# NethermindEth/starkpack-winterfell

Hardware: AMD Instinct MI355X
Metric: trace-LDE + Merkle-commit field-ops/s (wall-clock ms in ms_per_step), 2^20x8 f64 trace blowup=8 (higher is better)
Workload: dtype u64 (Goldilocks, Montgomery form) + u32 (BLAKE3)

## Files before the change

### starkpack-winterfell_amd/csrc/context.hip

```cpp
#include "wf_internal.hpp"

#include <atomic>

#include "field.hpp"

using namespace wf;

static thread_local char g_err[512] = "";

std::atomic<uint64_t> g_fail_epoch{0};
uint64_t fail_epoch() { return g_fail_epoch.load(std::memory_order_relaxed); }

int fail(int code, const char *fmt, ...) {
    g_fail_epoch.fetch_add(1, std::memory_order_relaxed);
    va_list ap;
    va_start(ap, fmt);
    vsnprintf(g_err, sizeof(g_err), fmt, ap);
    va_end(ap);
    return code;
}

const char *last_error_text() { return g_err; }

wf_tuning tuning_from_env() {
// ... 2 lines not shown
    if (!on || strcmp(on, "1") != 0) return t;
    if (const char *e = getenv("WF_EXP_MAX_DIGIT")) {
        const int v = atoi(e);
        if (v >= 4 && v <= 11) t.max_digit = (uint32_t)v;
    }
    t.no_specialized = getenv("WF_EXP_NO_SPECIALIZED") != nullptr;
    t.full_tiles = getenv("WF_EXP_FULL_TILES") != nullptr;
    t.no_fused_hash = getenv("WF_EXP_NO_FUSED_HASH") != nullptr;
    t.no_chunked = getenv("WF_EXP_NO_CHUNKED") != nullptr;
    t.persistent_always = getenv("WF_EXP_PERSISTENT_ALWAYS") != nullptr;
    t.no_persistent = getenv("WF_EXP_NO_PERSISTENT") != nullptr;
    if (const char *e = getenv("WF_EXP_MERKLE_L2_MIN")) {
        const int v = atoi(e);
        if (v >= 10 && v <= 30) t.merkle_l2_min = (uint32_t)v;
    }
    t.no_pipeline = getenv("WF_EXP_NO_PIPELINE") != nullptr;
    t.no_tail_pack = getenv("WF_EXP_NO_TAIL_PACK") != nullptr;
    t.no_coset_inner = getenv("WF_EXP_NO_COSET_INNER") != nullptr;
    t.no_gtab = getenv("WF_EXP_NO_GTAB") != nullptr;
    t.no_staged_chunks = getenv("WF_EXP_NO_STAGED_CHUNKS") != nullptr;
    t.no_gtab1 = getenv("WF_EXP_NO_GTAB1") != nullptr;
    t.no_ftab = getenv("WF_EXP_NO_FTAB") != nullptr;
    t.no_gtab1_wide = getenv("WF_EXP_NO_GTAB1_WIDE") != nullptr;
    t.gtab1_f64 = getenv("WF_EXP_GTAB1_F64") != nullptr;
    if (const char *e = getenv("WF_EXP_WIDE_TI")) {
        const int v = atoi(e);
        if (v == 1 || v == 2 || v == 4 || v == 8) t.wide_ti = (uint32_t)v;
    }
    if (const char *e = getenv("WF_EXP_PIPELINE_MIN_BYTES")) {
        const long long v = atoll(e);
        if (v >= 0 && v <= (1ll << 40)) t.pipeline_min_bytes = (size_t)v;
    }
    if (const char *e = getenv("WF_EXP_FAIL_AFTER_SEGMENT")) {
        const int v = atoi(e);
        if (v >= 0 && v < 4096) t.fail_after_segment = v;
    }
    if (const char *e = getenv("WF_EXP_GRIND_WINDOW_LOG2")) {
        const int v = atoi(e);
        if (v >= 2 && v <= 30) t.grind_window_log2 = (uint32_t)v;
    }
    if (const char *e = getenv("WF_EXP_GRIND_WINDOW_CAP_LOG2")) {
        const int v = atoi(e);
        if (v >= 2 && v <= 30) t.grind_window_cap_log2 = (uint32_t)v;
    }
    return t;
}
// ... 395 lines not shown
```

### starkpack-winterfell_amd/csrc/path.hip

```cpp
#include "wf_internal.hpp"

#include "kernels.hpp"
#include "keccak_dev.hpp"
#include "keccak_kernels.hpp"
#include "merkle_plan.hpp"
#include "rescue_kernels.hpp"
#include "rescue_jive_kernels.hpp"
#include "griffin_dev.hpp"
#include "seg_kernels.hpp"
#include "col_kernels.hpp"
#include "fri_kernels.hpp"
#include "tables.hpp"

using namespace wf;

#if defined(WF_EXPERIMENTS) && defined(WF_EXP_STAMPS)
static unsigned long long *g_exp_stamps = nullptr;
static unsigned long long *exp_stamps_buffer() {
    if (!g_exp_stamps && hipMalloc(&g_exp_stamps, 4096 * 8 * 8) == hipSuccess) (void)hipMemset(g_exp_stamps, 0, 4096 * 8 * 8);
    return g_exp_stamps;
}
extern "C" int wf_exp_stamps_read(unsigned long long *out, int clear) {
    if (!g_exp_stamps) return -1;
    if (hipMemcpy(out, g_exp_stamps, 4096 * 8 * 8, hipMemcpyDeviceToHost) != hipSuccess) return -2;
// ... 181 lines not shown
    return true;
}

template <class F>
struct SegDesc {
    typedef typename F::T T;
    const T *in;
    T *work;
    T *out;
    uint32_t logN, n_seg, n_cosets;
    bool rows_out;
    void *leaves = nullptr;
    uint32_t hash_epr = 0;
    uint32_t digest_words = 8;
    bool *fused = nullptr;
    const TableSet *pre;
    const T *fin_tab = nullptr;
    bool pad_traces = false;
    bool pad_in_kernel = false;
    uint32_t base_cols, total_base_cols, coset0;
    uint64_t row_width, trace_lde_elems;
    uint32_t seg0 = 0, seg_cnt = 0;
    int phase = 0;
};

template <class F>
static int run_seg_transform(wf_ctx *ctx, hipStream_t st, const SegDesc<F> &d) {
    typedef typename F::T T;
    const bool inverse = !d.rows_out;
    TableSet *tw;
    int rc = root_tables<F>(ctx, d.logN, inverse, &tw);
    if (rc) return rc;
    const Plan plan = seg_plan<F>(d.logN, d.n_seg, ctx->tune.max_digit, ctx->tune.full_tiles);
    const uint64_t N = (uint64_t)1 << d.logN;

    SegArgs<F> a;
    memset(&a, 0, sizeof(a));
    a.logN = d.logN;
    a.n_seg = d.n_seg;
    a.n_cosets = d.n_cosets;
    a.tw = as_pow2l<F>(*tw);
    if (d.pre) {
        a.pre = as_pow2l<F>(*d.pre);
        a.pre_lo_stride = d.pre->lo_stride;
        a.pre_hi_stride = d.pre->hi_stride;
    }
    a.base_cols = d.base_cols;
// ... 59 lines not shown
            a.dst = d.work;
            a.src_shared = 0;
            a.pre_on = 0;
            a.scale_on = first ? 1 : 0;
            a.scale = inv_n;
        }
        a.src += run_off;
        a.dst += run_off;
        a.n_seg = run_cnt;
        uint32_t threads;
        size_t lds;
        rc = seg_launch_dims<F>(a.logD, threads, lds, false);
        if (rc) return rc;
        const uint64_t grid = (uint64_t)n_groups * run_cnt * a.O * a.I;
        if (grid > 0x7FFFFFFFull) return fail(WF_ERR_ARG, "problem too large for one launch (%llu groups)", (unsigned long long)grid);
        auto coset_inner = [&](uint32_t cosets, uint64_t tiles_per_coset) -> uint32_t {
            if (!(d.rows_out && first) || ctx->tune.no_coset_inner || cosets < 2 || (cosets & (cosets - 1)) || (tiles_per_coset & 63)) return 0u;
            uint32_t lc = 0;
            while ((1u << lc) < cosets) lc++;
            return lc + 1;
        };
        prof_mark(ctx, st, tag_s);
        const bool spec_ok = F::BYTES == 8 && !packed && threads * 2 == (1u << a.logD) && !ctx->tune.no_specialized;
        const void *kern = nullptr;
        if (spec_ok) {
            constexpr bool F8 = F::BYTES == 8;
            switch (a.logD) {
                case 10: kern = d.rows_out ? (const void *)k_seg_strided<F, 1, false, F8 ? 10 : 0> : (const void *)k_seg_strided<F, 0, false, F8 ? 10 : 0>; break;
                case 9: kern = d.rows_out ? (const void *)k_seg_strided<F, 1, false, F8 ? 9 : 0> : (const void *)k_seg_strided<F, 0, false, F8 ? 9 : 0>; break;
                default: break;
            }
        }
        uint32_t ti = 0;
        if (F::BYTES == 8 && !packed && plan.n_pass >= 3 && a.logD >= 4 && a.logD <= 8 && ctx->tune.wide_ti != 1) {
            ti = ctx->tune.wide_ti ? ctx->tune.wide_ti : 2u;
            while (ti > 1 && (ti > a.I || ((size_t)(ti * SegCfg<F>::S + 2 + ti) << a.logD) * sizeof(T) > 80 * 1024)) ti >>= 1;
            if (ti < 2 || ((1u << a.logD) * ti * SegCfg<F>::S) / 16 < 64) ti = 0;
        }
        a.coset_inner = coset_inner(n_groups, ((uint64_t)run_cnt * a.O * a.I) / (ti ? ti : 1u));
        a.fout_tab = nullptr;
        if (!ti && d.rows_out && first && !packed && a.pre_on && !a.scale_on && d.logN <= 20 && !ctx->tune.no_gtab1 &&
            (F::BYTES == 16 || ctx->tune.gtab1_f64)) {
            rc = pass_factor_table<F>(ctx, d.logN, a.logD, (uint32_t)(d.logN - a.logD), inverse, &a.fout_tab);
            if (rc) return rc;
        }
        if (ti) {
// ... 166 lines not shown
            int rcq = ensure_tickets(ctx, st);
            if (rcq) return rcq;
            a.tile_counters = (uint32_t *)ctx->tickets.p;
#if defined(WF_EXPERIMENTS) && defined(WF_EXP_STAMPS)
            a.stamps = exp_stamps_buffer();
#endif
            void *kargs[] = {&a};
            HIP_TRY(hipLaunchKernel(kern, dim3((uint32_t)std::min<uint64_t>(tickets, resident)), dim3(threads), kargs, lds_p, st));
            if (chunked) {
                HIP_TRY(hipGetLastError());
                launch_merge_chunks(st, ctx->hash_tmp.p, n_chunks, launch_rows, d.leaves, a.digest_words);
            }
        } else if (d.rows_out && packed)
            hipLaunchKernelGGL((k_seg_last<F, SEG_OUT_ROWS, true>), dim3((uint32_t)grid), dim3(threads), lds, st, a);
        else {
            const void *kern = d.rows_out ? (const void *)k_seg_last<F, SEG_OUT_ROWS> : (const void *)k_seg_last<F, SEG_OUT_SEG>;
            constexpr bool F8 = F::BYTES == 8;
            if (F8 && threads * 2 == (1u << a.logD) && !ctx->tune.no_specialized) {
                if (a.logD == 10)
                    kern = d.rows_out ? (const void *)k_seg_last<F, SEG_OUT_ROWS, false, F8 ? 10 : 0> : (const void *)k_seg_last<F, SEG_OUT_SEG, false, F8 ? 10 : 0>;
                else if (a.logD == 9)
                    kern = d.rows_out ? (const void *)k_seg_last<F, SEG_OUT_ROWS, false, F8 ? 9 : 0> : (const void *)k_seg_last<F, SEG_OUT_SEG, false, F8 ? 9 : 0>;
            }
            if (lds > 64 * 1024) HIP_TRY(hipFuncSetAttribute(kern, hipFuncAttributeMaxDynamicSharedMemorySize, 160 * 1024));
            void *kargs[] = {&a};
            HIP_TRY(hipLaunchKernel(kern, dim3((uint32_t)grid), dim3(threads), kargs, lds, st));
        }
        HIP_TRY(hipGetLastError());
    }
    return 0;
}

template <class F>
static int run_xpose(wf_ctx *ctx, hipStream_t st, bool to_seg, const void *src, void *dst, uint64_t R, uint32_t W,
                     uint32_t total_base_cols, uint32_t n_seg, uint32_t seg0 = 0, uint32_t seg_cnt = 0) {
    if (seg_cnt == 0) seg_cnt = n_seg - seg0;
    XposeArgs<F> x;
    x.seg0 = seg0;
    x.src = (const typename F::T *)src;
    x.dst = (typename F::T *)dst;
    x.R = R;
    x.W = W;
    x.total_base_cols = total_base_cols;
    constexpr uint32_t RPB = XPOSE_TILES * 256 / SegCfg<F>::S;
    const uint64_t grid = (uint64_t)seg_cnt * ((R + RPB - 1) / RPB);
    if (grid > 0x7FFFFFFFull) return fail(WF_ERR_ARG, "problem too large for one launch");
// ... 205 lines not shown
    if (d_leaves) {
        if (!hashed) {
            prof_mark(ctx, st, "hash_rows");
            rc = run_hash_rows<F>(ctx, st, d_lde, Nrows * row_width, Nrows, (uint32_t)row_width, base_cols, p->n_traces, d_leaves, p->hasher, p->digest_bytes);
            if (rc) return rc;
        }
        if (d_nodes) {
            prof_mark(ctx, st, "merkle");
            rc = run_merkle(ctx, st, d_leaves, Nrows, d_nodes, p->hasher, p->digest_bytes);
            if (rc) return rc;
        }
    }
    prof_mark(ctx, st, "between_calls");
    return 0;
}

template <class F>
static int trace_commit_dev(wf_ctx *ctx, const wf_params *p, const void *d_trace, void *d_polys, void *d_lde,
                            void *d_leaves, void *d_nodes, hipStream_t st, hipEvent_t input_read = nullptr) {
    PathBufs<F> b;
    int rc = path_buffers<F>(ctx, p, b);
    if (rc) return rc;
    const uint64_t R = (uint64_t)1 << p->log2_trace_len;
    rc = run_xpose<F>(ctx, st, true, d_trace, b.segA, R, p->ext_degree, b.total_base_cols, b.n_seg);
    if (rc) return rc;
    if (input_read) HIP_TRY(hipEventRecord(input_read, st));
    SegDesc<F> d;
    memset(&d, 0, sizeof(d));
    d.in = b.segA;
    d.work = b.segA;
    d.out = b.segB;
    d.logN = p->log2_trace_len;
    d.n_seg = b.n_seg;
    d.n_cosets = 1;
    d.rows_out = false;
    rc = run_seg_transform<F>(ctx, st, d);
    if (rc) return rc;
    rc = run_xpose<F>(ctx, st, false, b.segB, d_polys, R, p->ext_degree, b.total_base_cols, b.n_seg);
    if (rc) return rc;
    return evaluate_and_commit<F>(ctx, st, p, b, d_lde, d_leaves, d_nodes);
}

template <class F>
static int trace_commit_pipelined_impl(wf_ctx *ctx, const wf_params *p, const void *const *cols_in, void *d_stage, void *d_polys,
                                       void *d_lde, void *d_leaves, void *d_nodes, hipStream_t st, void *const *polys_out) {
    typedef typename F::T T;
    constexpr uint32_t S = SegCfg<F>::S;
    PathBufs<F> b;
    int rc = path_buffers<F>(ctx, p, b);
    if (rc) return rc;
    const uint64_t R = (uint64_t)1 << p->log2_trace_len;
    const size_t colb = R * sizeof(T), TC = b.total_base_cols;
    if (!ctx->copy_stream) HIP_TRY(hipStreamCreateWithFlags(&ctx->copy_stream, hipStreamNonBlocking));
    while (ctx->seg_events.size() < (size_t)b.n_seg + 1) {
        hipEvent_t e;
        HIP_TRY(hipEventCreateWithFlags(&e, hipEventDisableTiming));
        ctx->seg_events.push_back(e);
    }
// ... 591 lines not shown
```

### starkpack-winterfell_amd/csrc/seg_kernels.hpp

```cpp
#pragma once

#include <hip/hip_runtime.h>
#include <stdint.h>

#include "field.hpp"
#include "kernels.hpp"

#ifndef WF_EXPERIMENTS
#undef WF_EXP_SKIP_LOAD
#undef WF_EXP_SKIP_NTT
#undef WF_EXP_SKIP_STORE
#undef WF_EXP_LOCAL_STORE
#undef WF_EXP_STAMPS
#endif

namespace wf {

template <class F>
struct SegCfg {
    static constexpr uint32_t S = 64 / F::BYTES;
    static constexpr uint32_t HP = S / 2;
    static constexpr bool RADIX16 = F::BYTES == 8;
    static constexpr bool RADIX8 = F::BYTES == 16;
    static constexpr uint32_t LOAD_BATCH = F::BYTES == 8 ? 8 : 4;
// ... 540 lines not shown
        T w8[4];
#pragma unroll
        for (int j = 0; j < 4; j++) w8[j] = twd[j * (D >> 3)];
        for (uint32_t r = radix8_rounds(logD); r > 0; r--) {
            seg_round8<F, LANES>(x, twd, w8, logD, cur, nthr, threadIdx.x);
            cur -= 3;
            __syncthreads();
        }
    }
    T w4 = F::one();
    if (logD >= 2) w4 = twd[D >> 2];
    while (cur > 0) {
        if (cur >= 2) {
            seg_round4<F, DIR, false, LANES>(x, twd, w4, logD, cur, nthr, threadIdx.x);
            cur -= 2;
        } else {
            seg_round2<F, LANES>(x, logD, nthr, threadIdx.x);
            cur = 0;
        }
        __syncthreads();
    }
}

template <class F, int EVAL, bool PACKED = false, int LOGD = 0>
__global__ void WF_TILE_BOUNDS(LOGD, 1024) k_seg_strided(SegArgs<F> a) {
    typedef typename F::T T;
    if (LOGD) a.logD = LOGD;
    const uint32_t NT = tile_threads<LOGD>();
    typedef Pair<T> P2;
    constexpr uint32_t S = SegCfg<F>::S, HP = SegCfg<F>::HP;
    constexpr uint32_t hp_shift = HP == 4 ? 2 : 1;
    extern __shared__ __attribute__((aligned(16))) unsigned char smem_raw[];
    const uint32_t D = 1u << a.logD;
    T *x = reinterpret_cast<T *>(smem_raw);
    T *twd = x + (size_t)D * S;
    constexpr bool ONE_TABLE = F::BYTES == 16;
    T *aux = ONE_TABLE ? twd : twd + D;

    uint64_t bid = xcd_group_index(blockIdx.x, gridDim.x);
    const uint32_t logI = ilog2_pow2(a.I), logO = ilog2_pow2(a.O);
    uint32_t c_in = 0;
    if (a.coset_inner) bid = coset_inner_split(bid, a.coset_inner - 1, c_in);
    const uint64_t i = bid & (a.I - 1);
    const uint64_t o = (bid >> logI) & (a.O - 1);
    const uint32_t rest = (uint32_t)(bid >> (logI + logO));
    const uint32_t c = a.coset_inner ? c_in : rest / a.n_seg, g = a.coset_inner ? rest : rest - c * a.n_seg;
    const uint64_t seg_elems = ((uint64_t)1 << a.logN) * S;
    const T *src = a.src + (a.src_shared ? (uint64_t)g : (uint64_t)c * a.seg_stride + g) * seg_elems;
    T *dst = a.dst + ((uint64_t)c * a.seg_stride + g) * seg_elems;

    Pow2L<F> pre = a.pre;
    Pow2L<F> pre_a = a.pre, pre_b = a.pre;
    const uint32_t lane_a = 2 * (threadIdx.x & (HP - 1)), lane_b = lane_a + 1;
    const bool act_a = PACKED && (lane_a & ((1u << a.lg_log) - 1)) < a.total_base_cols && (lane_a >> a.lg_log) < (1u << a.cpr_log);
    const bool act_b = PACKED && (lane_b & ((1u << a.lg_log) - 1)) < a.total_base_cols && (lane_b >> a.lg_log) < (1u << a.cpr_log);
    if (PACKED && a.pre_on) {
        const uint32_t ca = a.coset0 + (c << a.cpr_log) + (act_a ? (lane_a >> a.lg_log) : 0);
        const uint32_t cb = a.coset0 + (c << a.cpr_log) + (act_b ? (lane_b >> a.lg_log) : 0);
        pre_a.lo += (uint64_t)ca * a.pre_lo_stride;
        pre_a.hi += (uint64_t)ca * a.pre_hi_stride;
        pre_b.lo += (uint64_t)cb * a.pre_lo_stride;
        pre_b.hi += (uint64_t)cb * a.pre_hi_stride;
    } else if (a.pre_on) {
        pre.lo += (uint64_t)(a.coset0 + c) * a.pre_lo_stride;
        pre.hi += (uint64_t)(a.coset0 + c) * a.pre_hi_stride;
    }
    const uint32_t nitems = D * HP;
    const uint64_t row0 = ((o << a.logD) << logI) + i;
    const uint32_t step = NT;
    const bool from_regs = !(PACKED && a.pre_on);
    const uint32_t tw_shift = a.logN - a.logD - logI;
    const bool scale_in = !PACKED && a.pre_on;
    const Pow2L<F> pin = scale_in ? pre : a.tw;
    const bool gtab = !PACKED && a.fout_tab != nullptr;
    uint32_t kq[2];
    T fo_a[2], fo_b[2], tw_q[2], fi_a[2], fi_b[2];
#pragma unroll
    for (uint32_t q = 0; q < 2; q++) {
        const uint32_t k = threadIdx.x + q * NT;
        kq[q] = k < D ? k : D - 1;
        if (gtab)
            fo_a[q] = fo_b[q] = a.fout_tab[(i << a.logD) + kq[q]];
        else
            a.tw.fetch(((uint64_t)kq[q] * i) << tw_shift, fo_a[q], fo_b[q]);
        tw_q[q] = a.digit_tw[kq[q]];
        pin.fetch(((uint64_t)kq[q] << logI) + (gtab ? i : 0), fi_a[q], fi_b[q]);
    }
    const bool direct = !PACKED && SegCfg<F>::RADIX16 && a.logD >= 4 && from_regs;
    const uint32_t m16 = D >> 4, l16 = threadIdx.x & (S - 1), j16 = threadIdx.x / S;
    const bool has16 = threadIdx.x < m16 * S;
    T vr[16];
    uint4 r0, r1, r2, r3, r4, r5, r6, r7;
    r0 = r1 = r2 = r3 = r4 = r5 = r6 = r7 = make_uint4(0, 0, 0, 0);
    if (direct) {
        if (has16) {
            const T *pr = src + (row0 + ((uint64_t)j16 << logI)) * S + l16;
            const uint64_t rstep = ((uint64_t)m16 << logI) * S;
#pragma unroll
            for (uint32_t q = 0; q < 16; q++) {
#ifdef WF_EXP_SKIP_LOAD
                vr[q] = src[l16];
#else
                vr[q] = *pr;
#endif
                pr += rstep;
            }
        }
    } else if (from_regs) {
#ifdef WF_EXP_SKIP_LOAD
#define WF_ITEM_PTR(WK) reinterpret_cast<const uint4 *>(src + 2 * ((WK) & (HP - 1)))
#else
#define WF_ITEM_PTR(WK) \
    reinterpret_cast<const uint4 *>(src + (row0 + ((uint64_t)((WK) >> hp_shift) << logI)) * S + 2 * ((WK) & (HP - 1)))
#endif
#define WF_LOAD_ITEM(U, RA, RB)                            \
    do {                                                   \
        const uint32_t wk_ = threadIdx.x + (U) * step;     \
        if (wk_ < nitems) {                                \
            const uint4 *p_ = WF_ITEM_PTR(wk_);            \
            RA = p_[0];                                    \
// ... 104 lines not shown
#ifndef WF_EXP_SKIP_NTT
    seg_lds_ntt<F, EVAL ? 1 : -1, (LOGD ? (1u << LOGD) : 0u)>(x, twd, a.logD, NT, direct ? vr : nullptr, direct);
#else
    if (direct && has16) {
#pragma unroll
        for (uint32_t q = 0; q < 16; q++) x[(q * m16 + j16) * S + l16] = vr[q];
    }
    __syncthreads();
#endif
    if (ONE_TABLE) {
        if (threadIdx.x < D) aux[threadIdx.x] = unpark<F>(fok0);
        if (threadIdx.x + NT < D) aux[threadIdx.x + NT] = unpark<F>(fok1);
        __syncthreads();
    }

    T start_a = F::one(), start_b = F::one();
    if (PACKED && a.pre_on) {
        start_a = pre_a.get(i);
        start_b = pre_b.get(i);
    }
    const uint32_t pstride = NT >> hp_shift, pos0 = threadIdx.x >> hp_shift;
    if (pos0 >= D) return;
    const uint32_t k0 = seg_digit_reverse<F>(pos0, a.logD);
    T *dst_lane = dst + row0 * S + lane_a;
    const uint32_t k_shift = logI + (S == 8 ? 3 : 2);
    for (uint32_t pj = 0; pj < D; pj += pstride) {
        const uint32_t k = k0 | seg_digit_reverse<F>(pj, a.logD);
        P2 v = *reinterpret_cast<P2 *>(x + (pos0 + pj) * S + lane_a);
        const T f = aux[k];
        v.a = F::mul(v.a, f);
        v.b = F::mul(v.b, f);
        if (PACKED && a.pre_on) {
            v.a = F::mul(v.a, start_a);
            v.b = F::mul(v.b, start_b);
        }
#ifdef WF_EXP_SKIP_STORE
        if (*reinterpret_cast<const uint32_t *>(&v.a) == a.logN + 77777u)
#endif
        store_pair(dst_lane + ((uint64_t)k << k_shift), v);
    }
}

template <class F, int EVAL, int TI, int GTAB = 0, int LOGD = 0>
__global__ void __launch_bounds__(1024) k_seg_strided_wide(SegArgs<F> a) {
    if (LOGD) a.logD = LOGD;
    static_assert(SegCfg<F>::RADIX16 && TI >= 2 && (TI & (TI - 1)) == 0, "f64 tiles of 2, 4 or 8 inner positions");
    typedef typename F::T T;
    typedef Pair<T> P2;
    constexpr uint32_t S = SegCfg<F>::S, LANES = TI * S, HPW = LANES / 2;
    constexpr uint32_t LOGS = ilog2_const(S), LOGL = ilog2_const(LANES), LOGTI = ilog2_const(TI), LOGHPW = ilog2_const(HPW);
    extern __shared__ __attribute__((aligned(16))) unsigned char smem_raw[];
    const uint32_t D = 1u << a.logD, NT = blockDim.x;
    T *x = reinterpret_cast<T *>(smem_raw);
    T *twd = x + (size_t)D * LANES;
    T *fin = twd + D;
    T *fout = fin + D;

    uint64_t bid = xcd_group_index(blockIdx.x, gridDim.x);
    uint32_t c_in = 0;
    if (a.coset_inner) bid = coset_inner_split(bid, a.coset_inner - 1, c_in);
    const uint32_t logI = ilog2_pow2(a.I), logO = ilog2_pow2(a.O), logIt = logI - LOGTI;
    const uint64_t i0 = (bid & ((a.I >> LOGTI) - 1)) << LOGTI;
    const uint64_t o = (bid >> logIt) & (a.O - 1);
// ... 155 lines not shown
    if (psub >= pstep) return;
    for (uint32_t t = lo / bc; t <= (hi - 1) / bc; t++) {
        const uint32_t b0 = t * bc + s2, b1 = b0 + 1, last = t * bc + bc - 1;
        const bool d0 = s2 < bc, d1 = s2 + 1 < bc;
        const bool pad_here = last >= lo && last < hi;
        const bool in0 = d0 ? (b0 >= lo && b0 < hi) : pad_here, in1 = d1 ? (b1 >= lo && b1 < hi) : pad_here;
        if (!in0 && !in1) continue;
        T *row = a.dst + (uint64_t)t * a.trace_lde_elems + (uint64_t)c * a.row_width + s2;
        for (uint32_t pos = psub; pos < D; pos += pstep) {
            const uint64_t k = rev_o + ((uint64_t)seg_digit_reverse<F>(pos, a.logD) << out_shift);
            const uint64_t off = (uint64_t)(uint32_t)k * k_stride;
            const T v0 = d0 && in0 ? x[pos * S + (b0 - lo)] : F::zero();
            const T v1 = d1 && in1 ? x[pos * S + (b1 - lo)] : F::zero();
            if (in0 && in1)
                store_pair(row + off, Pair<T>{v0, v1});
            else if (in0)
                row[off] = v0;
            else
                row[off + 1] = v1;
        }
    }
}

template <class F, int OUT, bool PACKED = false, int LOGD = 0>
__global__ void WF_TILE_BOUNDS(LOGD, 1024) k_seg_last(SegArgs<F> a) {
    typedef typename F::T T;
    const uint32_t logD_ = LOGD ? (uint32_t)LOGD : a.logD;
    const uint32_t NT = tile_threads<LOGD>();
    typedef Pair<T> P2;
    constexpr uint32_t S = SegCfg<F>::S, HP = SegCfg<F>::HP;
    constexpr uint32_t hp_shift = HP == 4 ? 2 : 1;
    extern __shared__ __attribute__((aligned(16))) unsigned char smem_raw[];
    const uint32_t D = 1u << logD_;
    T *x = reinterpret_cast<T *>(smem_raw);
    T *twd = x + (size_t)D * S;
    T *aux = twd;

    uint64_t bid = xcd_group_index(blockIdx.x, gridDim.x);
    const uint32_t logO = ilog2_pow2(a.O);
    const uint32_t b32 = (uint32_t)bid;
    const uint32_t q32 = b32 / a.n_cosets, c = b32 - q32 * a.n_cosets;
    const uint64_t o = q32 & (uint32_t)(a.O - 1);
    const uint32_t g = q32 >> logO;
    const uint64_t seg_elems = ((uint64_t)1 << a.logN) * S;
    const T *src = a.src + (a.src_shared ? (uint64_t)g : (uint64_t)c * a.n_seg + g) * seg_elems + (o << logD_) * S;

    uint64_t rev_o = 0;
    {
        uint32_t bits = 0;
        for (uint32_t q = 0; q < a.n_prev; q++) bits += a.prev_log[q];
        uint32_t hi = bits, sh = 0;
        for (uint32_t q = 0; q < a.n_prev; q++) {
            hi -= a.prev_log[q];
            rev_o |= ((o >> hi) & (((uint64_t)1 << a.prev_log[q]) - 1)) << sh;
            sh += a.prev_log[q];
        }
    }

    Pow2L<F> pre = a.pre, pre_a = a.pre, pre_b = a.pre;
    const uint32_t lane_a = 2 * (threadIdx.x & (HP - 1)), lane_b = lane_a + 1;
    const bool act_a = PACKED && (lane_a & ((1u << a.lg_log) - 1)) < a.total_base_cols && (lane_a >> a.lg_log) < (1u << a.cpr_log);
    const bool act_b = PACKED && (lane_b & ((1u << a.lg_log) - 1)) < a.total_base_cols && (lane_b >> a.lg_log) < (1u << a.cpr_log);
    if (PACKED && a.pre_on) {
        const uint32_t ca = a.coset0 + (c << a.cpr_log) + (act_a ? (lane_a >> a.lg_log) : 0);
        const uint32_t cb = a.coset0 + (c << a.cpr_log) + (act_b ? (lane_b >> a.lg_log) : 0);
        pre_a.lo += (uint64_t)ca * a.pre_lo_stride;
        pre_a.hi += (uint64_t)ca * a.pre_hi_stride;
        pre_b.lo += (uint64_t)cb * a.pre_lo_stride;
// ... 16 lines not shown
        tw_q[q] = a.digit_tw[kq[q]];
        if (!PACKED && a.fin_tab)
            fi_a[q] = fi_b[q] = a.fin_tab[((uint64_t)(a.coset0 + c) << a.logN) + kq[q]];
        else
            pin.fetch(kq[q], fi_a[q], fi_b[q]);
    }
    const uint4 twk0 = park(tw_q[0]), twk1 = park(tw_q[1]);
    uint4 r0, r1, r2, r3, r4, r5, r6, r7;
    r0 = r1 = r2 = r3 = r4 = r5 = r6 = r7 = make_uint4(0, 0, 0, 0);
#ifdef WF_EXP_SKIP_LOAD
#define WF_ITEM_PTR(WK) reinterpret_cast<const uint4 *>(a.src + 2 * (uint64_t)((WK) & 63))
#else
#define WF_ITEM_PTR(WK) reinterpret_cast<const uint4 *>(src + 2 * (uint64_t)(WK))
#endif
#define WF_LOAD_ITEM(U, RA, RB)                            \
    do {                                                   \
        const uint32_t wk_ = threadIdx.x + (U) * step;     \
        if (wk_ < nitems) {                                \
            const uint4 *p_ = WF_ITEM_PTR(wk_);            \
            RA = p_[0];                                    \
            if (F::BYTES == 16) RB = p_[1];                \
        }                                                  \
    } while (0)
    if (from_regs) {
        if (F::BYTES == 8) {
            WF_LOAD_ITEM(0, r0, r0);
            WF_LOAD_ITEM(1, r1, r1);
            WF_LOAD_ITEM(2, r2, r2);
            WF_LOAD_ITEM(3, r3, r3);
            WF_LOAD_ITEM(4, r4, r4);
            WF_LOAD_ITEM(5, r5, r5);
            WF_LOAD_ITEM(6, r6, r6);
            WF_LOAD_ITEM(7, r7, r7);
        } else {
            WF_LOAD_ITEM(0, r0, r1);
            WF_LOAD_ITEM(1, r2, r3);
            WF_LOAD_ITEM(2, r4, r5);
            WF_LOAD_ITEM(3, r6, r7);
        }
    }
#undef WF_LOAD_ITEM
#undef WF_ITEM_PTR
#pragma unroll
    for (uint32_t q = 0; q < 2; q++) {
        if (threadIdx.x + q * NT < D) {
            if (scale_in)
                aux[kq[q]] = (!PACKED && a.fin_tab) ? fi_a[q] : F::mul(fi_a[q], fi_b[q]);
            else
                twd[kq[q]] = unpark<F>(q == 0 ? twk0 : twk1);
        }
    }
    __syncthreads();
    if (PACKED && a.pre_on) {
        for (uint32_t wk = threadIdx.x; wk < nitems; wk += NT) {
            P2 v;
            const uint32_t d = wk >> hp_shift;
            const uint32_t lgm = (1u << a.lg_log) - 1, cola = lane_a & lgm, colb = lane_b & lgm;
            const T *srow = src + (uint64_t)d * S;
            const T fa = pre_a.get(d);
            const T fb = a.lg_log ? fa : pre_b.get(d);
            v.a = act_a ? F::mul(srow[cola], fa) : F::zero();
            v.b = act_b ? F::mul(srow[colb], fb) : F::zero();
            *reinterpret_cast<P2 *>(x + 2 * wk) = v;
        }
    } else {
#define WF_FILL_ITEM(U, RA, RB)                                \
    do {                                                       \
        const uint32_t wk_ = threadIdx.x + (U) * step;         \
        if (wk_ < nitems) {                                    \
            P2 v_ = pair_from<F>(RA, RB);                      \
            if (a.pre_on) {                                    \
                const T f_ = aux[wk_ >> hp_shift];             \
                v_.a = F::mul(v_.a, f_);                       \
                v_.b = F::mul(v_.b, f_);                       \
            }                                                  \
            *reinterpret_cast<P2 *>(x + 2 * wk_) = v_;         \
// ... 148 lines not shown
                dl[1] = digest_hi(out[4], out[5], out[6], out[7], a.digest_words);
            }
        }
    }
    if (OUT == SEG_OUT_ROWS && !PACKED && a.leaves) {
        constexpr uint32_t WPE = F::BYTES / 4;
        for (uint32_t pos = threadIdx.x; pos < D; pos += NT) {
            T ev[S];
            uint4 *evq = reinterpret_cast<uint4 *>(ev);
            const uint4 *q = reinterpret_cast<const uint4 *>(x + (size_t)pos * S);
#pragma unroll
            for (uint32_t w = 0; w < 4; w++) evq[w] = q[w];
            uint32_t m[16], out[8];
#pragma unroll
            for (uint32_t e = 0; e < S; e++) elem_words<F>(ev[e], &m[e * WPE]);
            b3::set_iv(out);
            b3::compress(out, m, 0, 0, a.hash_epr * F::BYTES, b3::CHUNK_START | b3::CHUNK_END | b3::ROOT);
            const uint64_t k = rev_o + ((uint64_t)seg_digit_reverse<F>(pos, logD_) << (a.logN - logD_));
            uint4 *dl = reinterpret_cast<uint4 *>(a.leaves + ((uint64_t)(uint32_t)k * a.rows_per_k + c) * 8);
            dl[0] = make_uint4(out[0], out[1], out[2], out[3]);
            dl[1] = digest_hi(out[4], out[5], out[6], out[7], a.digest_words);
        }
    }
}


template <class F, bool MULTI, bool PADT = false, bool CHUNKED = false, bool SMALL = false, int LOGD = 0>
__global__ void __launch_bounds__((LOGD) ? (1 << ((LOGD) ? (LOGD) - 1 : 0)) : (SMALL ? 256 : 1024), ((LOGD) || (SMALL && PADT && CHUNKED)) ? 4 : 1)
k_seg_last_hash(SegArgs<F> a) {
    typedef typename F::T T;
    const uint32_t logD_ = LOGD ? (uint32_t)LOGD : a.logD;
    const uint32_t NT = tile_threads<LOGD>();
    typedef Pair<T> P2;
    constexpr uint32_t S = SegCfg<F>::S, HP = SegCfg<F>::HP;
    constexpr uint32_t hp_shift = HP == 4 ? 2 : 1;
    constexpr uint32_t WPE = F::BYTES / 4;
    extern __shared__ __attribute__((aligned(16))) unsigned char smem_raw[];
    const uint32_t D = 1u << logD_;
    T *x = reinterpret_cast<T *>(smem_raw);
    T *twd = x + (size_t)D * S;
    const uint32_t n_chunks = CHUNKED ? a.n_chunks : 1;
    const uint64_t total = (uint64_t)a.n_cosets * a.O * n_chunks;
    const uint64_t seg_elems = ((uint64_t)1 << a.logN) * S;
    const uint32_t step = NT;
    const uint32_t out_shift = a.logN - logD_;
    const uint32_t k_stride = a.rows_per_k * (uint32_t)a.row_width;
// ... 568 lines not shown
```

### starkpack-winterfell_amd/csrc/tables.hpp

```cpp
#pragma once

#include "wf_internal.hpp"

#include "pow2l.hpp"

using namespace wf;

static int table_upload(wf_ctx *ctx, void **dst, const void *src, size_t bytes) {
    *dst = nullptr;
    hipError_t e = dev_malloc(ctx, dst, bytes);
    if (e != hipSuccess) return fail(WF_ERR_HIP, "table allocation of %zu bytes failed: %s", bytes, hipGetErrorString(e));
    e = hipMemcpy(*dst, src, bytes, hipMemcpyHostToDevice);
    if (e != hipSuccess) {
        (void)hipFree(*dst);
        *dst = nullptr;
        return fail(WF_ERR_HIP, "table upload failed: %s", hipGetErrorString(e));
    }
    return 0;
}

template <class F>
static int upload_pow2l(wf_ctx *ctx, const std::vector<typename F::T> &bases, uint32_t logN, TableSet &ts) {
    typedef typename F::T T;
    const uint32_t s = (logN + 1) / 2;
// ... 174 lines not shown
        if (inverse) w = f_inv<F>(w);
        const uint64_t D = (uint64_t)1 << logD, I = (uint64_t)1 << logI;
        const T base = f_pow<F>(w, (u128)1 << (logN - logD - logI));
        std::vector<T> tab(D * I);
        T step = F::one();
        for (uint64_t i = 0; i < I; i++) {
            T acc = F::one();
            for (uint64_t k = 0; k < D; k++) {
                tab[i * D + k] = acc;
                acc = F::mul(acc, step);
            }
            step = F::mul(step, base);
        }
        TableSet ts;
        const int rcu = table_upload(ctx, &ts.lo, tab.data(), tab.size() * sizeof(T));
        if (rcu) return rcu;
        it = ctx->tables.emplace(key, ts).first;
    }
    *out = (const typename F::T *)it->second.lo;
    return 0;
}

template <class F>
static typename F::T offset_elem(const wf_params *p, uint64_t &lo, uint64_t &hi) {
    u128 off;
    memcpy(&off, p->domain_offset, 16);
    lo = (uint64_t)off;
    hi = (uint64_t)(off >> 64);
    return F::from_u128_canonical(off);
}
```

### starkpack-winterfell_amd/csrc/wf_internal.hpp

```cpp
#pragma once

#include "../../include/wf_lde.h"

#include <hip/hip_runtime.h>

#include <algorithm>
#include <atomic>
#include <cstdarg>
#include <cstdio>
#include <cstring>
#include <map>
#include <mutex>
#include <set>
#include <string>
#include <thread>
#include <tuple>
#include <type_traits>
#include <vector>

int fail(int code, const char *fmt, ...) __attribute__((format(printf, 2, 3)));
const char *last_error_text();
uint64_t fail_epoch();

#define HIP_TRY(expr)                                                                              \
// ... 12 lines not shown
    uint32_t s = 0, mask = 0;
    uint64_t lo_stride = 0, hi_stride = 0;
};

struct wf_tuning {
    uint32_t max_digit = 0;
    bool full_tiles = false;
    bool no_specialized = false;
    bool no_fused_hash = false;
    bool no_chunked = false;
    bool persistent_always = false;
    bool no_persistent = false;
    uint32_t merkle_l2_min = 18;
    bool no_pipeline = false;
    size_t pipeline_min_bytes = (size_t)1 << 20;
    bool no_tail_pack = false;
    bool no_coset_inner = false;
    bool no_gtab1_wide = false;
    bool no_ftab = false;
    bool no_gtab1 = false;
    bool gtab1_f64 = false;
    bool no_staged_chunks = false;
    bool no_gtab = false;
    uint32_t wide_ti = 0;
    int fail_after_segment = -1;
    uint32_t grind_window_log2 = 0;
    uint32_t grind_window_cap_log2 = 0;
};
wf_tuning tuning_from_env();

struct wf_ctx {
    int device = 0;
    int num_cus = 256;
    wf_tuning tune;
    uint32_t digest_bytes = 32;
    uint32_t hasher = WF_HASH_BLAKE3;
    DevBuf pack_tmp;
    hipStream_t stream = nullptr;
    std::map<std::tuple<int, int, int, int, uint64_t, uint64_t>, TableSet> tables;
    int prof_level = 0;
    bool prof_on = false;
    std::vector<hipEvent_t> prof_ev;
    std::vector<const char *> prof_name;
    size_t prof_n = 0;
    DevBuf scratch;
    DevBuf io[5];
// ... 181 lines not shown
```

Baseline: 1971 billion.

## Read column-major trace directly in interpolation passes, skipping the input transpose

For base-field traces whose segmented plan has two passes, the inverse NTT now reads columns straight from the column-major input instead of first running a transpose kernel into segment layout. New column-tile variants of the strided and last-pass kernels load column data and scatter results using a precomputed table that folds together the twiddle factors and the 1/N normalization. This removes one full read and write of the trace. In exchange, loads become strided and there is an extra factor table of N elements.

```diff
diff --git a/starkpack-winterfell_amd/csrc/context.hip b/starkpack-winterfell_amd/csrc/context.hip
--- a/starkpack-winterfell_amd/csrc/context.hip
+++ b/starkpack-winterfell_amd/csrc/context.hip
@@ -48,6 +48,7 @@
     t.no_gtab1 = getenv("WF_EXP_NO_GTAB1") != nullptr;
     t.no_ftab = getenv("WF_EXP_NO_FTAB") != nullptr;
     t.no_gtab1_wide = getenv("WF_EXP_NO_GTAB1_WIDE") != nullptr;
+    t.no_col_tiles = getenv("WF_EXP_NO_COL_TILES") != nullptr;
     t.gtab1_f64 = getenv("WF_EXP_GTAB1_F64") != nullptr;
     if (const char *e = getenv("WF_EXP_WIDE_TI")) {
         const int v = atoi(e);
diff --git a/starkpack-winterfell_amd/csrc/path.hip b/starkpack-winterfell_amd/csrc/path.hip
--- a/starkpack-winterfell_amd/csrc/path.hip
+++ b/starkpack-winterfell_amd/csrc/path.hip
@@ -227,7 +227,16 @@
     uint64_t row_width, trace_lde_elems;
     uint32_t seg0 = 0, seg_cnt = 0;
     int phase = 0;
+    bool col_tiles = false;
+    hipEvent_t input_read = nullptr;
 };
+
+template <class F>
+static bool col_tiles_ok(const wf_ctx *ctx, uint32_t logN, uint32_t n_seg) {
+    if (F::BYTES != 8 || ctx->tune.no_col_tiles) return false;
+    const Plan plan = seg_plan<F>(logN, n_seg, ctx->tune.max_digit, ctx->tune.full_tiles);
+    return plan.n_pass == 2 && plan.dig[0] >= 4 && plan.dig[1] >= 3;
+}
 
 template <class F>
 static int run_seg_transform(wf_ctx *ctx, hipStream_t st, const SegDesc<F> &d) {
@@ -333,6 +342,24 @@
         };
         prof_mark(ctx, st, tag_s);
         const bool spec_ok = F::BYTES == 8 && !packed && threads * 2 == (1u << a.logD) && !ctx->tune.no_specialized;
+        if (d.col_tiles) {
+            if constexpr (F::BYTES == 8) {
+                rc = col_tile_factor_table<F>(ctx, d.logN, a.logD, &a.fout_tab);
+                if (rc) return rc;
+                a.total_base_cols = d.total_base_cols;
+                const uint64_t grid_c = (uint64_t)d.total_base_cols * (a.I >> 3);
+                if (grid_c > 0x7FFFFFFFull) return fail(WF_ERR_ARG, "problem too large for one launch (%llu groups)", (unsigned long long)grid_c);
+                const void *kc = spec_ok && a.logD == 10 ? (const void *)k_seg_strided_cols<F, 10>
+                               : spec_ok && a.logD == 9  ? (const void *)k_seg_strided_cols<F, 9>
+                                                         : (const void *)k_seg_strided_cols<F>;
+                if (lds > 64 * 1024) HIP_TRY(hipFuncSetAttribute(kc, hipFuncAttributeMaxDynamicSharedMemorySize, 160 * 1024));
+                void *kargs[] = {&a};
+                HIP_TRY(hipLaunchKernel(kc, dim3((uint32_t)grid_c), dim3(threads), kargs, lds, st));
+                if (d.input_read) HIP_TRY(hipEventRecord(d.input_read, st));
+            }
+            done_bits += a.logD;
+            continue;
+        }
         const void *kern = nullptr;
         if (spec_ok) {
             constexpr bool F8 = F::BYTES == 8;
@@ -545,6 +572,14 @@
                 else if (a.logD == 9)
                     kern = d.rows_out ? (const void *)k_seg_last<F, SEG_OUT_ROWS, false, F8 ? 9 : 0> : (const void *)k_seg_last<F, SEG_OUT_SEG, false, F8 ? 9 : 0>;
             }
+            if (d.col_tiles) {
+                if constexpr (F8) {
+                    const bool spec = threads * 2 == (1u << a.logD) && !ctx->tune.no_specialized;
+                    kern = spec && a.logD == 10 ? (const void *)k_seg_last_cols<F, 10>
+                         : spec && a.logD == 9  ? (const void *)k_seg_last_cols<F, 9>
+                                                : (const void *)k_seg_last_cols<F>;
+                }
+            }
             if (lds > 64 * 1024) HIP_TRY(hipFuncSetAttribute(kern, hipFuncAttributeMaxDynamicSharedMemorySize, 160 * 1024));
             void *kargs[] = {&a};
             HIP_TRY(hipLaunchKernel(kern, dim3((uint32_t)grid), dim3(threads), kargs, lds, st));
@@ -796,18 +831,26 @@
     int rc = path_buffers<F>(ctx, p, b);
     if (rc) return rc;
     const uint64_t R = (uint64_t)1 << p->log2_trace_len;
-    rc = run_xpose<F>(ctx, st, true, d_trace, b.segA, R, p->ext_degree, b.total_base_cols, b.n_seg);
-    if (rc) return rc;
-    if (input_read) HIP_TRY(hipEventRecord(input_read, st));
+    const bool col_tiles = p->ext_degree == 1 && col_tiles_ok<F>(ctx, p->log2_trace_len, b.n_seg);
+    if (!col_tiles) {
+        rc = run_xpose<F>(ctx, st, true, d_trace, b.segA, R, p->ext_degree, b.total_base_cols, b.n_seg);
+        if (rc) return rc;
+        if (input_read) HIP_TRY(hipEventRecord(input_read, st));
+    }
     SegDesc<F> d;
     memset(&d, 0, sizeof(d));
-    d.in = b.segA;
+    d.in = col_tiles ? (const typename F::T *)d_trace : b.segA;
     d.work = b.segA;
     d.out = b.segB;
     d.logN = p->log2_trace_len;
     d.n_seg = b.n_seg;
     d.n_cosets = 1;
     d.rows_out = false;
+    d.col_tiles = col_tiles;
+    if (col_tiles) {
+        d.total_base_cols = b.total_base_cols;
+        d.input_read = input_read;
+    }
     rc = run_seg_transform<F>(ctx, st, d);
     if (rc) return rc;
     rc = run_xpose<F>(ctx, st, false, b.segB, d_polys, R, p->ext_degree, b.total_base_cols, b.n_seg);
diff --git a/starkpack-winterfell_amd/csrc/seg_kernels.hpp b/starkpack-winterfell_amd/csrc/seg_kernels.hpp
--- a/starkpack-winterfell_amd/csrc/seg_kernels.hpp
+++ b/starkpack-winterfell_amd/csrc/seg_kernels.hpp
@@ -586,8 +586,8 @@
     }
 }
 
-template <class F, int EVAL, bool PACKED = false, int LOGD = 0>
-__global__ void WF_TILE_BOUNDS(LOGD, 1024) k_seg_strided(SegArgs<F> a) {
+template <class F, int EVAL, bool PACKED, int LOGD, bool COLS>
+__device__ __forceinline__ void seg_strided_tile(SegArgs<F> a) {
     typedef typename F::T T;
     if (LOGD) a.logD = LOGD;
     const uint32_t NT = tile_threads<LOGD>();
@@ -605,11 +605,11 @@
     const uint32_t logI = ilog2_pow2(a.I), logO = ilog2_pow2(a.O);
     uint32_t c_in = 0;
     if (a.coset_inner) bid = coset_inner_split(bid, a.coset_inner - 1, c_in);
-    const uint64_t i = bid & (a.I - 1);
-    const uint64_t o = (bid >> logI) & (a.O - 1);
-    const uint32_t rest = (uint32_t)(bid >> (logI + logO));
-    const uint32_t c = a.coset_inner ? c_in : rest / a.n_seg, g = a.coset_inner ? rest : rest - c * a.n_seg;
-    const uint64_t seg_elems = ((uint64_t)1 << a.logN) * S;
+    const uint64_t i = COLS ? (bid & ((a.I >> 3) - 1)) << 3 : bid & (a.I - 1);
+    const uint64_t o = COLS ? 0 : (bid >> logI) & (a.O - 1);
+    const uint32_t rest = (uint32_t)(bid >> (COLS ? logI - 3 : logI + logO));
+    const uint32_t c = COLS ? 0 : a.coset_inner ? c_in : rest / a.n_seg, g = a.coset_inner ? rest : rest - c * a.n_seg;
+    const uint64_t seg_elems = ((uint64_t)1 << a.logN) * (COLS ? 1 : S);
     const T *src = a.src + (a.src_shared ? (uint64_t)g : (uint64_t)c * a.seg_stride + g) * seg_elems;
     T *dst = a.dst + ((uint64_t)c * a.seg_stride + g) * seg_elems;
 
@@ -636,21 +636,23 @@
     const uint32_t tw_shift = a.logN - a.logD - logI;
     const bool scale_in = !PACKED && a.pre_on;
     const Pow2L<F> pin = scale_in ? pre : a.tw;
-    const bool gtab = !PACKED && a.fout_tab != nullptr;
+    const bool gtab = !COLS && !PACKED && a.fout_tab != nullptr;
     uint32_t kq[2];
     T fo_a[2], fo_b[2], tw_q[2], fi_a[2], fi_b[2];
 #pragma unroll
     for (uint32_t q = 0; q < 2; q++) {
         const uint32_t k = threadIdx.x + q * NT;
         kq[q] = k < D ? k : D - 1;
-        if (gtab)
+        if (COLS)
+            fo_a[q] = fo_b[q] = F::one();
+        else if (gtab)
             fo_a[q] = fo_b[q] = a.fout_tab[(i << a.logD) + kq[q]];
         else
             a.tw.fetch(((uint64_t)kq[q] * i) << tw_shift, fo_a[q], fo_b[q]);
         tw_q[q] = a.digit_tw[kq[q]];
         pin.fetch(((uint64_t)kq[q] << logI) + (gtab ? i : 0), fi_a[q], fi_b[q]);
     }
-    const bool direct = !PACKED && SegCfg<F>::RADIX16 && a.logD >= 4 && from_regs;
+    const bool direct = COLS || (!PACKED && SegCfg<F>::RADIX16 && a.logD >= 4 && from_regs);
     const uint32_t m16 = D >> 4, l16 = threadIdx.x & (S - 1), j16 = threadIdx.x / S;
     const bool has16 = threadIdx.x < m16 * S;
     T vr[16];
@@ -658,8 +660,8 @@
     r0 = r1 = r2 = r3 = r4 = r5 = r6 = r7 = make_uint4(0, 0, 0, 0);
     if (direct) {
         if (has16) {
-            const T *pr = src + (row0 + ((uint64_t)j16 << logI)) * S + l16;
-            const uint64_t rstep = ((uint64_t)m16 << logI) * S;
+            const T *pr = COLS ? src + ((uint64_t)j16 << logI) + i + l16 : src + (row0 + ((uint64_t)j16 << logI)) * S + l16;
+            const uint64_t rstep = ((uint64_t)m16 << logI) * (COLS ? 1 : S);
 #pragma unroll
             for (uint32_t q = 0; q < 16; q++) {
 #ifdef WF_EXP_SKIP_LOAD
@@ -810,6 +812,51 @@
     const uint32_t pstride = NT >> hp_shift, pos0 = threadIdx.x >> hp_shift;
     if (pos0 >= D) return;
     const uint32_t k0 = seg_digit_reverse<F>(pos0, a.logD);
+    if constexpr (COLS) {
+        const uint64_t lane0 = i + lane_a;
+        if constexpr (LOGD != 0 && F::BYTES == 8) {
+            uint4 f0, f1, f2, f3, f4, f5, f6, f7;
+#define WF_COLS_AT(J) (((uint64_t)(k0 | seg_digit_reverse<F>((J) * pstride, a.logD)) << logI) + lane0)
+#define WF_COLS_LOAD(J, R) R = *reinterpret_cast<const uint4 *>(a.fout_tab + WF_COLS_AT(J))
+#define WF_COLS_STORE(J, R)                                                              \
+    do {                                                                                 \
+        P2 v_ = *reinterpret_cast<P2 *>(x + (pos0 + (J) * pstride) * S + lane_a);        \
+        const P2 f_ = pair_from<F>(R, R);                                                \
+        v_.a = F::mul(v_.a, f_.a);                                                       \
+        v_.b = F::mul(v_.b, f_.b);                                                       \
+        store_pair(dst + WF_COLS_AT(J), v_);                                             \
+    } while (0)
+            WF_COLS_LOAD(0, f0);
+            WF_COLS_LOAD(1, f1);
+            WF_COLS_LOAD(2, f2);
+            WF_COLS_LOAD(3, f3);
+            WF_COLS_LOAD(4, f4);
+            WF_COLS_LOAD(5, f5);
+            WF_COLS_LOAD(6, f6);
+            WF_COLS_LOAD(7, f7);
+            WF_COLS_STORE(0, f0);
+            WF_COLS_STORE(1, f1);
+            WF_COLS_STORE(2, f2);
+            WF_COLS_STORE(3, f3);
+            WF_COLS_STORE(4, f4);
+            WF_COLS_STORE(5, f5);
+            WF_COLS_STORE(6, f6);
+            WF_COLS_STORE(7, f7);
+#undef WF_COLS_STORE
+#undef WF_COLS_LOAD
+#undef WF_COLS_AT
+            return;
+        }
+        for (uint32_t pj = 0; pj < D; pj += pstride) {
+            const uint64_t at = ((uint64_t)(k0 | seg_digit_reverse<F>(pj, a.logD)) << logI) + lane0;
+            P2 v = *reinterpret_cast<P2 *>(x + (pos0 + pj) * S + lane_a);
+            const P2 f = *reinterpret_cast<const P2 *>(a.fout_tab + at);
+            v.a = F::mul(v.a, f.a);
+            v.b = F::mul(v.b, f.b);
+            store_pair(dst + at, v);
+        }
+        return;
+    }
     T *dst_lane = dst + row0 * S + lane_a;
     const uint32_t k_shift = logI + (S == 8 ? 3 : 2);
     for (uint32_t pj = 0; pj < D; pj += pstride) {
@@ -827,6 +874,16 @@
 #endif
         store_pair(dst_lane + ((uint64_t)k << k_shift), v);
     }
+}
+
+template <class F, int EVAL, bool PACKED = false, int LOGD = 0>
+__global__ void WF_TILE_BOUNDS(LOGD, 1024) k_seg_strided(SegArgs<F> a) {
+    seg_strided_tile<F, EVAL, PACKED, LOGD, false>(a);
+}
+
+template <class F, int LOGD = 0>
+__global__ void WF_TILE_BOUNDS(LOGD, 1024) k_seg_strided_cols(SegArgs<F> a) {
+    seg_strided_tile<F, 0, false, LOGD, true>(a);
 }
 
 template <class F, int EVAL, int TI, int GTAB = 0, int LOGD = 0>
@@ -1028,8 +1085,8 @@
     }
 }
 
-template <class F, int OUT, bool PACKED = false, int LOGD = 0>
-__global__ void WF_TILE_BOUNDS(LOGD, 1024) k_seg_last(SegArgs<F> a) {
+template <class F, int OUT, bool PACKED, int LOGD, bool COLS>
+__device__ __forceinline__ void seg_last_tile(const SegArgs<F> &a) {
     typedef typename F::T T;
     const uint32_t logD_ = LOGD ? (uint32_t)LOGD : a.logD;
     const uint32_t NT = tile_threads<LOGD>();
@@ -1049,7 +1106,7 @@
     const uint64_t o = q32 & (uint32_t)(a.O - 1);
     const uint32_t g = q32 >> logO;
     const uint64_t seg_elems = ((uint64_t)1 << a.logN) * S;
-    const T *src = a.src + (a.src_shared ? (uint64_t)g : (uint64_t)c * a.n_seg + g) * seg_elems + (o << logD_) * S;
+    const T *src = a.src + (a.src_shared ? (uint64_t)g : (uint64_t)c * a.n_seg + g) * seg_elems + (o << logD_) * (COLS ? 1 : S);
 
     uint64_t rev_o = 0;
     {
@@ -1112,7 +1169,23 @@
             if (F::BYTES == 16) RB = p_[1];                \
         }                                                  \
     } while (0)
-    if (from_regs) {
+    if (COLS) {
+        const uint32_t live = a.total_base_cols - g * S;
+        const uint64_t col_elems = (uint64_t)1 << a.logN;
+        if (2 * threadIdx.x < D) {
+#define WF_LOAD_COL(J, R) \
+    if ((J) < live) R = *reinterpret_cast<const uint4 *>(src + (J) * col_elems + 2 * threadIdx.x)
+            WF_LOAD_COL(0, r0);
+            WF_LOAD_COL(1, r1);
+            WF_LOAD_COL(2, r2);
+            WF_LOAD_COL(3, r3);
+            WF_LOAD_COL(4, r4);
+            WF_LOAD_COL(5, r5);
+            WF_LOAD_COL(6, r6);
+            WF_LOAD_COL(7, r7);
+#undef WF_LOAD_COL
+        }
+    } else if (from_regs) {
         if (F::BYTES == 8) {
             WF_LOAD_ITEM(0, r0, r0);
             WF_LOAD_ITEM(1, r1, r1);
@@ -1141,7 +1214,21 @@
         }
     }
     __syncthreads();
-    if (PACKED && a.pre_on) {
+    if (COLS) {
+        if constexpr (F::BYTES == 8) {
+            if (2 * threadIdx.x < D) {
+                uint4 *row = reinterpret_cast<uint4 *>(x + (size_t)(2 * threadIdx.x) * S);
+                row[0] = make_uint4(r0.x, r0.y, r1.x, r1.y);
+                row[1] = make_uint4(r2.x, r2.y, r3.x, r3.y);
+                row[2] = make_uint4(r4.x, r4.y, r5.x, r5.y);
+                row[3] = make_uint4(r6.x, r6.y, r7.x, r7.y);
+                row[4] = make_uint4(r0.z, r0.w, r1.z, r1.w);
+                row[5] = make_uint4(r2.z, r2.w, r3.z, r3.w);
+                row[6] = make_uint4(r4.z, r4.w, r5.z, r5.w);
+                row[7] = make_uint4(r6.z, r6.w, r7.z, r7.w);
+            }
+        }
+    } else if (PACKED && a.pre_on) {
         for (uint32_t wk = threadIdx.x; wk < nitems; wk += NT) {
             P2 v;
             const uint32_t d = wk >> hp_shift;
@@ -1336,6 +1423,16 @@
             dl[1] = digest_hi(out[4], out[5], out[6], out[7], a.digest_words);
         }
     }
+}
+
+template <class F, int OUT, bool PACKED = false, int LOGD = 0>
+__global__ void WF_TILE_BOUNDS(LOGD, 1024) k_seg_last(SegArgs<F> a) {
+    seg_last_tile<F, OUT, PACKED, LOGD, false>(a);
+}
+
+template <class F, int LOGD = 0>
+__global__ void WF_TILE_BOUNDS(LOGD, 1024) k_seg_last_cols(SegArgs<F> a) {
+    seg_last_tile<F, SEG_OUT_SEG, false, LOGD, true>(a);
 }
 
 
diff --git a/starkpack-winterfell_amd/csrc/tables.hpp b/starkpack-winterfell_amd/csrc/tables.hpp
--- a/starkpack-winterfell_amd/csrc/tables.hpp
+++ b/starkpack-winterfell_amd/csrc/tables.hpp
@@ -220,6 +220,34 @@
 }
 
 template <class F>
+static int col_tile_factor_table(wf_ctx *ctx, uint32_t logN, uint32_t logD, const typename F::T **out) {
+    auto key = std::make_tuple((int)F::FIELD_ID, (int)logN, 9, (int)logD, (uint64_t)0, (uint64_t)0);
+    auto it = ctx->tables.find(key);
+    if (it == ctx->tables.end()) {
+        typedef typename F::T T;
+        const T w = f_inv<F>(f_root_of_unity<F>(logN ? logN : 1));
+        const T inv_n = f_inv<F>(F::from_u128_canonical((u128)1 << logN));
+        const uint64_t D = (uint64_t)1 << logD, I = (uint64_t)1 << (logN - logD);
+        std::vector<T> tab(D * I);
+        T step = F::one();
+        for (uint64_t k = 0; k < D; k++) {
+            T acc = inv_n;
+            for (uint64_t i = 0; i < I; i++) {
+                tab[k * I + i] = acc;
+                acc = F::mul(acc, step);
+            }
+            step = F::mul(step, w);
+        }
+        TableSet ts;
+        const int rcu = table_upload(ctx, &ts.lo, tab.data(), tab.size() * sizeof(T));
+        if (rcu) return rcu;
+        it = ctx->tables.emplace(key, ts).first;
+    }
+    *out = (const typename F::T *)it->second.lo;
+    return 0;
+}
+
+template <class F>
 static typename F::T offset_elem(const wf_params *p, uint64_t &lo, uint64_t &hi) {
     u128 off;
     memcpy(&off, p->domain_offset, 16);
diff --git a/starkpack-winterfell_amd/csrc/wf_internal.hpp b/starkpack-winterfell_amd/csrc/wf_internal.hpp
--- a/starkpack-winterfell_amd/csrc/wf_internal.hpp
+++ b/starkpack-winterfell_amd/csrc/wf_internal.hpp
@@ -58,6 +58,7 @@
     bool gtab1_f64 = false;
     bool no_staged_chunks = false;
     bool no_gtab = false;
+    bool no_col_tiles = false;
     uint32_t wide_ti = 0;
     int fail_after_segment = -1;
     uint32_t grind_window_log2 = 0;
```

New measurement: 2013 billion (median of 6 runs). 2.2% higher.
